# bxh1/VIDO-SLAM

Hardware: AMD Instinct MI355X
Metric: frames/sec end-to-end (flow+depth+track+local-BA) at 640x480; BA iters/sec (higher is better)
Workload: dtype f32

## Files before the change

vido-slam_amd/csrc/conv3x3h.hip:

```cpp
#include "common.hpp"
#include <type_traits>

namespace {
typedef float f32x16 __attribute__((ext_vector_type(16)));
typedef float f32x2 __attribute__((ext_vector_type(2)));
typedef _Float16 f16x8 __attribute__((ext_vector_type(8)));
typedef _Float16 f16x2 __attribute__((ext_vector_type(2)));
typedef unsigned u32x4 __attribute__((ext_vector_type(4)));

#define C3_OOB 0x40000000u
#define C3_WSLOT 24576
#define C3_RBW 3
#define C3_WPIX(BR) (((BR) + 2) * 18)
#define C3_XP(BR) ((16 * C3_WPIX(BR) + 511) / 512)
#define C3_RAW(BR) (C3_XP(BR) * 8 * 256)
#define C3_PLANE(BR) (C3_WPIX(BR) * 32)
#define C3_PBUF(BR) (2 * C3_PLANE(BR))
#define C3_LDS(BR) (C3_RBW * C3_WSLOT + C3_RAW(BR) + 2 * C3_PBUF(BR))

struct C3Args { const float* x; const void* wp; const float* bias; float* y; int N, Cin, Cout, H, W, nby, nbx, mt, total, nchunk; float slope; unsigned wbytes; unsigned* range_flag; };

template <int RPW, int CG>
__global__ __launch_bounds__(512) void k_conv3x3_h(C3Args A)
{
    constexpr int BR = 16 / CG, MT = 32 * RPW * CG, WPIX = C3_WPIX(BR), XP = C3_XP(BR), RAWB = C3_RAW(BR), PLANE = C3_PLANE(BR), PBUF = C3_PBUF(BR), CK = (WPIX * 8 + 511) / 512, NMM = 9 * RPW, NRD = 2 * RPW + 2;
    extern __shared__ __attribute__((aligned(16))) char c3_lds[];
    char* L = c3_lds;
    const int tid = threadIdx.x, lane = tid & 63, w = __builtin_amdgcn_readfirstlane(tid >> 6);
    const int per = gridDim.x >> 3, item = (blockIdx.x & 7) * per + (blockIdx.x >> 3);
    if (item >= A.total) return;
    const int nt = item / A.mt, mtile = item - nt * A.mt, m0 = mtile * MT;
    const int bpi = A.nby * A.nbx, n = nt / bpi, brem = nt - n * bpi, by = brem / A.nbx, bx = brem - by * A.nbx, Y0 = by * BR, X0 = bx * 16;
    const int rp = CG == 1 ? w : (w & 3), rb0 = CG == 1 ? 0 : RPW * (w >> 2);
    const int hw = A.H * A.W, nsteps = A.nchunk * 3;

    const __amdgpu_buffer_rsrc_t wr = __builtin_amdgcn_make_buffer_rsrc((void*)A.wp, 0, A.wbytes, 0x00020000);
    const unsigned avo = 16u * (unsigned)lane;
    unsigned abase[3], avq[3];
#pragma unroll
    for (int q = 0; q < 3; q++) { const int i = w + 8 * q, rb = i / 6, rem = i - 6 * rb; abase[q] = 1024u * (unsigned)(((m0 >> 5) + rb) * A.nchunk * 18 + rem); avq[q] = rb < RPW * CG ? avo : 0x80000000u; }
    unsigned xvo[11];
#pragma unroll
    for (int j = 0; j < XP; j++) {
        const int e = 64 * (8 * j + w) + lane, ch = e / WPIX, rem = e - ch * WPIX, row = rem / 18, col = rem - row * 18, gy = Y0 - 1 + row, gx = X0 - 1 + col;
        xvo[j] = (e < 16 * WPIX && gy >= 0 && gy < A.H && gx >= 0 && gx < A.W) ? 4u * (unsigned)(ch * hw + gy * A.W + gx) : C3_OOB;
    }
    const unsigned ximg = 4u * (unsigned)n * (unsigned)A.Cin * (unsigned)hw, ximg_end = ximg + 4u * (unsigned)A.Cin * (unsigned)hw, xchunk = 64u * (unsigned)hw;
    char* const RAW = L + C3_RBW * C3_WSLOT;
    char* const PL = RAW + RAWB;
    auto issue_w = [&](int s, int slot) {
        char* S = L + slot * C3_WSLOT + w * 1024;
        const unsigned so = 6144u * (unsigned)s;
#pragma unroll
        for (int q = 0; q < 3; q++) __builtin_amdgcn_raw_ptr_buffer_load_lds(wr, (__attribute__((address_space(3))) void*)(S + q * 8192), 16, avq[q], abase[q] + so, 0, 0);
    };
    auto issue_x = [&](int c) {
        const unsigned so = ximg + xchunk * (unsigned)c;
        const __amdgpu_buffer_rsrc_t xc = __builtin_amdgcn_make_buffer_rsrc((void*)((const char*)A.x + so), 0, ximg_end - so, 0x00020000);
#pragma unroll
        for (int j = 0; j < XP; j++) __builtin_amdgcn_raw_ptr_buffer_load_lds(xc, (__attribute__((address_space(3))) void*)(RAW + (8 * j + w) * 256), 4, xvo[j], 0, 0, 0);
    };
    float xmax = 0.f;
    const f32x2 k2048 = {2048.f, 2048.f};
    auto convert = [&](int buf) {
        const float* R = (const float*)RAW;
        unsigned* P = (unsigned*)(PL + buf * PBUF);
#pragma unroll
        for (int k = 0; k < CK; k++) {
            const int idx = tid + 512 * k;
            if (k < CK - 1 || idx < WPIX * 8) {
                const int q = idx / WPIX, pix = idx - q * WPIX;
                const f32x2 v = {R[(2 * q) * WPIX + pix], R[(2 * q + 1) * WPIX + pix]};
                const f16x2 h = __builtin_convertvector(v, f16x2);
                f32x2 vs, r;
                asm("v_pk_mul_f32 %0, %1, %2" : "=v"(vs) : "v"(v), "v"(k2048));
                asm("v_fma_mix_f32 %0, %1, %2, %3 op_sel_hi:[1,0,0]" : "=v"(r.x) : "v"(h), "s"(-2048.f), "v"(vs.x));
                asm("v_fma_mix_f32 %0, %1, %2, %3 op_sel:[1,0,0] op_sel_hi:[1,0,0]" : "=v"(r.y) : "v"(h), "s"(-2048.f), "v"(vs.y));
                const f16x2 l = __builtin_convertvector(r, f16x2);
                P[pix * 8 + q] = __builtin_bit_cast(unsigned, h); P[PLANE / 4 + pix * 8 + q] = __builtin_bit_cast(unsigned, l);
                xmax = __builtin_elementwise_maximum(__builtin_elementwise_maximum(xmax, __builtin_fabsf(v.x)), __builtin_fabsf(v.y));
            }
        }
    };

    f32x16 acc[RPW], acl[RPW];
#pragma unroll
    for (int rb = 0; rb < RPW; rb++)
#pragma unroll
        for (int r = 0; r < 16; r++) { acc[rb][r] = 0.f; acl[rb][r] = 0.f; }
    typedef const __attribute__((address_space(3))) char* lds_c;
    const unsigned a_lane = 16u * (unsigned)lane;
    const unsigned b_lane = (unsigned)(C3_RBW * C3_WSLOT + RAWB) + 32u * (unsigned)((2 * rp + ((lane & 31) >> 4)) * 18 + (lane & 15)) + 16u * (unsigned)(lane >> 5);

    issue_x(0); issue_w(0, 0); issue_w(min(1, nsteps - 1), 1);
    asm volatile("s_waitcnt vmcnt(6) lgkmcnt(0)\n\ts_barrier" ::: "memory");
    convert(0);
    int slot = 0;
    u32x4 a[2][RPW][2], b[2][2];
    auto step = [&](auto dy_c, auto nbuf_c, int pbuf, auto&& copies) {
        constexpr int dy = decltype(dy_c)::value, NBUF = decltype(nbuf_c)::value;
        lds_c Ab = (lds_c)(L + slot * C3_WSLOT) + a_lane;
        lds_c Bb = (lds_c)L + b_lane + pbuf * PBUF + dy * (18 * 32);
        auto ld = [&](int dx, int set) {
#pragma unroll
            for (int rb = 0; rb < RPW; rb++)
#pragma unroll
                for (int pl = 0; pl < 2; pl++) a[set][rb][pl] = *(const __attribute__((address_space(3))) u32x4*)(Ab + (((rb0 + rb) * 3 + dx) * 2 + pl) * 1024);
#pragma unroll
            for (int pl = 0; pl < 2; pl++) b[set][pl] = *(const __attribute__((address_space(3))) u32x4*)(Bb + dx * 32 + pl * PLANE);
        };
        __builtin_amdgcn_sched_barrier(0);
        ld(0, 0);
        copies();
#pragma unroll
        for (int dx = 0; dx < 3; dx++) {
            if (dx < 2) ld(dx + 1, (dx + 1) & 1);
#pragma unroll
            for (int term = 0; term < 3; term++) {
                constexpr int PA[3] = {0, 1, 0}, PB[3] = {1, 0, 0};
#pragma unroll
                for (int rb = 0; rb < RPW; rb++) {
                    f32x16& d = term == 2 ? acc[rb] : acl[rb];
                    d = __builtin_amdgcn_mfma_f32_32x32x16_f16(__builtin_bit_cast(f16x8, a[dx & 1][rb][PA[term]]), __builtin_bit_cast(f16x8, b[dx & 1][PB[term]]), d, 0, 0, 0);
                }
            }
        }
        __builtin_amdgcn_sched_group_barrier(0x100, NRD, 0);
#pragma unroll
        for (int i = 0; i < NMM; i++) {
            __builtin_amdgcn_sched_group_barrier(0x008, 1, 0);
            if (i < 2 * NRD) __builtin_amdgcn_sched_group_barrier(0x100, 1, 0);
            if (i >= 1 && i < 1 + NBUF) __builtin_amdgcn_sched_group_barrier(0x020, 1, 0);
        }
        __builtin_amdgcn_sched_barrier(0);
    };
    for (int c = 0; c < A.nchunk; c++) {
        const int pbuf = c & 1, cn = min(c + 1, A.nchunk - 1);
        asm volatile("s_waitcnt vmcnt(3) lgkmcnt(0)\n\ts_barrier" ::: "memory");
        step(std::integral_constant<int, 0>{}, std::integral_constant<int, 3 + XP>{}, pbuf, [&] { const int sf = slot == 0 ? C3_RBW - 1 : slot - 1; issue_w(min(3 * c + 2, nsteps - 1), sf); issue_x(cn); });
        slot = slot + 1 == C3_RBW ? 0 : slot + 1;
        asm volatile("s_waitcnt vmcnt(%0) lgkmcnt(0)\n\ts_barrier" :: "n"(3 + XP) : "memory");
        step(std::integral_constant<int, 1>{}, std::integral_constant<int, 3>{}, pbuf, [&] { const int sf = slot == 0 ? C3_RBW - 1 : slot - 1; issue_w(min(3 * c + 3, nsteps - 1), sf); });
        slot = slot + 1 == C3_RBW ? 0 : slot + 1;
        asm volatile("s_waitcnt vmcnt(3) lgkmcnt(0)\n\ts_barrier" ::: "memory");
        step(std::integral_constant<int, 2>{}, std::integral_constant<int, 3>{}, pbuf, [&] { const int sf = slot == 0 ? C3_RBW - 1 : slot - 1; issue_w(min(3 * c + 4, nsteps - 1), sf); });
        convert(pbuf ^ 1);
        slot = slot + 1 == C3_RBW ? 0 : slot + 1;
    }
    asm volatile("s_waitcnt vmcnt(0) lgkmcnt(0)" ::: "memory");
#pragma unroll
    for (int rb = 0; rb < RPW; rb++) acc[rb] += acl[rb] * 0x1p-11f;
    if (!(xmax < 65504.f) && A.range_flag) atomicOr(A.range_flag, 1u);

    const float* wsc = (const float*)((const char*)A.wp + (size_t)A.nchunk * 16 * 18 * A.Cout * 2);
    const int p = lane & 31, Y = Y0 + 2 * rp + (p >> 4), X = X0 + (p & 15);
    const bool inside = Y < A.H && X < A.W;
    float* yb = A.y + (size_t)n * A.Cout * hw + (size_t)Y * A.W + X;
#pragma unroll
    for (int rb = 0; rb < RPW; rb++) {
        float bv[16], sv[16];
#pragma unroll
        for (int r = 0; r < 16; r++) { const int co = m0 + 32 * (rb0 + rb) + 8 * (r >> 2) + 4 * (lane >> 5) + (r & 3); bv[r] = A.bias ? A.bias[co] : 0.f; sv[r] = wsc[co]; }
        if (inside) {
#pragma unroll
            for (int r = 0; r < 16; r++) {
                const int co = m0 + 32 * (rb0 + rb) + 8 * (r >> 2) + 4 * (lane >> 5) + (r & 3);
                const float v = acc[rb][r] * sv[r] + bv[r];
                yb[(size_t)co * hw] = fmaxf(v, v * A.slope);
            }
        }
    }
}
}

extern "C" {

int vido_conv3x3_h_supported(int n, int cin, int cout, int h, int w)
{
    const long long cp = (cin + 15) / 16 * 16;
    return n >= 1 && cin >= 1 && (cout == 32 || cout == 64 || (cout >= 128 && cout % 128 == 0)) && h >= 1 && w >= 1 && 4ll * n * cin * h * w < (1ll << 30) && 4ll * n * cout * h * w < (1ll << 30)
           && 36ll * cp * cout < (1ll << 31);
}

#define C3_MIN16 190
static int c3_block_rows(int n, int cout, int h, int w)
{
    static const int force = [] { const char* e = getenv("VIDO_CONV3X3_H_ROWS"); return e ? atoi(e) : 0; }();
    if (cout == 32) return 16;
    if (force == 16 || force == 8) return force;
    const int mt = cout >= 128 ? cout / 128 : 1;
    return n * ((h + 15) / 16) * ((w + 15) / 16) * mt >= C3_MIN16 ? 16 : 8;
}
int vido_conv3x3_h_workgroups(int n, int cout, int h, int w) { const int br = c3_block_rows(n, cout, h, w); return n * ((h + br - 1) / br) * ((w + 15) / 16) * (cout >= 128 ? cout / 128 : 1); }

int vido_conv3x3_h_bias_act(vido_ctx* ctx, const float* x, const void* w_packed, const float* bias, float* y, int n, int cin, int cout, int h, int w, float slope)
{
    if (!ctx) return VIDO_E_INVALID;
    if (!x || !w_packed || !y || x == y || !vido_conv3x3_h_supported(n, cin, cout, h, w) || slope < 0.f || slope > 1.f || (((uintptr_t)x | (uintptr_t)y) & 3) || ((uintptr_t)w_packed & 15))
        return vido_set_error(ctx, VIDO_E_INVALID, "conv3x3_h: no kernel for %d x %d -> %d channels at %d x %d (or a pointer is misaligned, or slope outside [0, 1])", n, cin, cout, h, w);
    HIP_TRY(ctx, hipSetDevice(ctx->device));
    hipStream_t st = ctx->has_ext_stream ? ctx->ext_stream : ctx->stream;
    const int br = c3_block_rows(n, cout, h, w);
    const int nby = (h + br - 1) / br, nbx = (w + 15) / 16, mt = cout >= 128 ? cout / 128 : 1, total = n * nby * nbx * mt;
    const int nchunk = (cin + 15) / 16;
    C3Args A{x, w_packed, bias, y, n, cin, cout, h, w, nby, nbx, mt, total, nchunk, slope, (unsigned)(36ll * 16 * nchunk * cout), ctx->c1_range_flag};
    static bool attr[64] = {};
    if (!attr[ctx->device & 63]) {
#define C3_ATTR(RPW_, CG_) HIP_TRY(ctx, hipFuncSetAttribute((const void*)k_conv3x3_h<RPW_, CG_>, hipFuncAttributeMaxDynamicSharedMemorySize, (int)C3_LDS(16 / CG_)))
        C3_ATTR(4, 1); C3_ATTR(2, 2); C3_ATTR(2, 1); C3_ATTR(1, 2); C3_ATTR(1, 1);
#undef C3_ATTR
        attr[ctx->device & 63] = true;
    }
    const dim3 grid(8 * ((total + 7) / 8));
#define C3_LAUNCH(RPW_, CG_) hipLaunchKernelGGL((k_conv3x3_h<RPW_, CG_>), grid, dim3(512), C3_LDS(16 / CG_), st, A)
    if (cout >= 128) { if (br == 16) C3_LAUNCH(4, 1); else C3_LAUNCH(2, 2); }
    else if (cout == 64) { if (br == 16) C3_LAUNCH(2, 1); else C3_LAUNCH(1, 2); }
    else C3_LAUNCH(1, 1);
#undef C3_LAUNCH
    HIP_TRY(ctx, hipGetLastError());
    return VIDO_OK;
}

}
```

Before: 125.0.

## Load conv input via registers and stage whole 3x3 weight chunks per slot

Input chunks no longer go through a raw f32 LDS staging area. They are loaded with buffer loads straight into registers and converted to the split f16 hi/lo planes, with 128-bit LDS stores. For the smaller output-tile variants the weight ring now holds all three dy rows of a chunk per slot, so a chunk needs one barrier instead of three. Ring depth is derived per template from an LDS budget. The aim is to cut LDS traffic, barriers and LDS footprint, at the cost of more registers held live across the MFMA loop and different waitcnt accounting.

Measured after the change: 127.2, median of 6. 1.7% higher.

```diff
diff --git a/vido-slam_amd/csrc/conv3x3h.hip b/vido-slam_amd/csrc/conv3x3h.hip
--- a/vido-slam_amd/csrc/conv3x3h.hip
+++ b/vido-slam_amd/csrc/conv3x3h.hip
@@ -9,21 +9,27 @@
 typedef unsigned u32x4 __attribute__((ext_vector_type(4)));
 
 #define C3_OOB 0x40000000u
-#define C3_WSLOT 24576
-#define C3_RBW 3
-#define C3_WPIX(BR) (((BR) + 2) * 18)
-#define C3_XP(BR) ((16 * C3_WPIX(BR) + 511) / 512)
-#define C3_RAW(BR) (C3_XP(BR) * 8 * 256)
-#define C3_PLANE(BR) (C3_WPIX(BR) * 32)
-#define C3_PBUF(BR) (2 * C3_PLANE(BR))
-#define C3_LDS(BR) (C3_RBW * C3_WSLOT + C3_RAW(BR) + 2 * C3_PBUF(BR))
+#ifndef C3_RING128
+#define C3_RING128 3
+#endif
+template <int RPW, int CG> struct C3Form {
+    static constexpr int BR = 16 / CG, RB = RPW * CG, DS = RB == 4 ? 1 : 3;
+    static constexpr int PPR = 6 * DS, QW = (RB * PPR + 7) / 8, WSLOT = 8 * QW * 1024;
+    static constexpr int WPIX = (BR + 2) * 18, PLANE = WPIX * 32, PBUF = 2 * PLANE;
+    static constexpr int XI = (2 * WPIX + 511) / 512, XL = 8 * XI;
+    static constexpr int RBW = DS == 1 ? C3_RING128 : (3 * WSLOT + 2 * PBUF <= 160 * 1024 ? 3 : 2);
+    static constexpr int LDS = RBW * WSLOT + 2 * PBUF;
+    static_assert(LDS <= 160 * 1024 && QW <= 5 && XI <= 2, "conv3x3_h: LDS, register arrays");
+};
 
 struct C3Args { const float* x; const void* wp; const float* bias; float* y; int N, Cin, Cout, H, W, nby, nbx, mt, total, nchunk; float slope; unsigned wbytes; unsigned* range_flag; };
 
 template <int RPW, int CG>
 __global__ __launch_bounds__(512) void k_conv3x3_h(C3Args A)
 {
-    constexpr int BR = 16 / CG, MT = 32 * RPW * CG, WPIX = C3_WPIX(BR), XP = C3_XP(BR), RAWB = C3_RAW(BR), PLANE = C3_PLANE(BR), PBUF = C3_PBUF(BR), CK = (WPIX * 8 + 511) / 512, NMM = 9 * RPW, NRD = 2 * RPW + 2;
+    typedef C3Form<RPW, CG> F;
+    constexpr int BR = F::BR, MT = 32 * RPW * CG, DS = F::DS, PPR = F::PPR, QW = F::QW, WSLOT = F::WSLOT, RBW = F::RBW, PD = RBW - 1;
+    constexpr int WPIX = F::WPIX, PLANE = F::PLANE, PBUF = F::PBUF, XI = F::XI, XL = F::XL, NMM = 9 * RPW, NRD = 2 * RPW + 2;
     extern __shared__ __attribute__((aligned(16))) char c3_lds[];
     char* L = c3_lds;
     const int tid = threadIdx.x, lane = tid & 63, w = __builtin_amdgcn_readfirstlane(tid >> 6);
@@ -32,53 +38,59 @@
     const int nt = item / A.mt, mtile = item - nt * A.mt, m0 = mtile * MT;
     const int bpi = A.nby * A.nbx, n = nt / bpi, brem = nt - n * bpi, by = brem / A.nbx, bx = brem - by * A.nbx, Y0 = by * BR, X0 = bx * 16;
     const int rp = CG == 1 ? w : (w & 3), rb0 = CG == 1 ? 0 : RPW * (w >> 2);
-    const int hw = A.H * A.W, nsteps = A.nchunk * 3;
+    const int hw = A.H * A.W, nsteps = A.nchunk * (3 / DS);
 
     const __amdgpu_buffer_rsrc_t wr = __builtin_amdgcn_make_buffer_rsrc((void*)A.wp, 0, A.wbytes, 0x00020000);
     const unsigned avo = 16u * (unsigned)lane;
-    unsigned abase[3], avq[3];
-#pragma unroll
-    for (int q = 0; q < 3; q++) { const int i = w + 8 * q, rb = i / 6, rem = i - 6 * rb; abase[q] = 1024u * (unsigned)(((m0 >> 5) + rb) * A.nchunk * 18 + rem); avq[q] = rb < RPW * CG ? avo : 0x80000000u; }
-    unsigned xvo[11];
-#pragma unroll
-    for (int j = 0; j < XP; j++) {
-        const int e = 64 * (8 * j + w) + lane, ch = e / WPIX, rem = e - ch * WPIX, row = rem / 18, col = rem - row * 18, gy = Y0 - 1 + row, gx = X0 - 1 + col;
-        xvo[j] = (e < 16 * WPIX && gy >= 0 && gy < A.H && gx >= 0 && gx < A.W) ? 4u * (unsigned)(ch * hw + gy * A.W + gx) : C3_OOB;
+    unsigned abase[5], avq[5];
+#pragma unroll
+    for (int q = 0; q < QW; q++) { const int i = w + 8 * q, rb = i / PPR, rem = i - PPR * rb; abase[q] = 1024u * (unsigned)(((m0 >> 5) + rb) * A.nchunk * 18 + rem); avq[q] = rb < RPW * CG ? avo : 0x80000000u; }
+    unsigned xo[2], xs[2];
+#pragma unroll
+    for (int k = 0; k < XI; k++) {
+        const int e = tid + 512 * k, hh = e / WPIX, pix = e - hh * WPIX, row = pix / 18, col = pix - row * 18, gy = Y0 - 1 + row, gx = X0 - 1 + col;
+        const bool in = hh < 2 && gy >= 0 && gy < A.H && gx >= 0 && gx < A.W;
+        xo[k] = in ? 4u * (unsigned)(8 * hh * hw + gy * A.W + gx) : C3_OOB; xs[k] = in ? 4u * (unsigned)hw : 0u;
     }
     const unsigned ximg = 4u * (unsigned)n * (unsigned)A.Cin * (unsigned)hw, ximg_end = ximg + 4u * (unsigned)A.Cin * (unsigned)hw, xchunk = 64u * (unsigned)hw;
-    char* const RAW = L + C3_RBW * C3_WSLOT;
-    char* const PL = RAW + RAWB;
+    char* const PL = L + RBW * WSLOT;
     auto issue_w = [&](int s, int slot) {
-        char* S = L + slot * C3_WSLOT + w * 1024;
-        const unsigned so = 6144u * (unsigned)s;
-#pragma unroll
-        for (int q = 0; q < 3; q++) __builtin_amdgcn_raw_ptr_buffer_load_lds(wr, (__attribute__((address_space(3))) void*)(S + q * 8192), 16, avq[q], abase[q] + so, 0, 0);
-    };
+        char* S = L + slot * WSLOT + w * 1024;
+        const unsigned so = 1024u * PPR * (unsigned)s;
+#pragma unroll
+        for (int q = 0; q < QW; q++) __builtin_amdgcn_raw_ptr_buffer_load_lds(wr, (__attribute__((address_space(3))) void*)(S + q * 8192), 16, avq[q], abase[q] + so, 0, 0);
+    };
+    float xv[2][8];
     auto issue_x = [&](int c) {
         const unsigned so = ximg + xchunk * (unsigned)c;
         const __amdgpu_buffer_rsrc_t xc = __builtin_amdgcn_make_buffer_rsrc((void*)((const char*)A.x + so), 0, ximg_end - so, 0x00020000);
 #pragma unroll
-        for (int j = 0; j < XP; j++) __builtin_amdgcn_raw_ptr_buffer_load_lds(xc, (__attribute__((address_space(3))) void*)(RAW + (8 * j + w) * 256), 4, xvo[j], 0, 0, 0);
+        for (int k = 0; k < XI; k++)
+#pragma unroll
+            for (int j = 0; j < 8; j++) xv[k][j] = __builtin_bit_cast(float, __builtin_amdgcn_raw_buffer_load_b32(xc, xo[k] + (unsigned)j * xs[k], 0, 0));
     };
     float xmax = 0.f;
     const f32x2 k2048 = {2048.f, 2048.f};
     auto convert = [&](int buf) {
-        const float* R = (const float*)RAW;
-        unsigned* P = (unsigned*)(PL + buf * PBUF);
-#pragma unroll
-        for (int k = 0; k < CK; k++) {
-            const int idx = tid + 512 * k;
-            if (k < CK - 1 || idx < WPIX * 8) {
-                const int q = idx / WPIX, pix = idx - q * WPIX;
-                const f32x2 v = {R[(2 * q) * WPIX + pix], R[(2 * q + 1) * WPIX + pix]};
-                const f16x2 h = __builtin_convertvector(v, f16x2);
-                f32x2 vs, r;
-                asm("v_pk_mul_f32 %0, %1, %2" : "=v"(vs) : "v"(v), "v"(k2048));
-                asm("v_fma_mix_f32 %0, %1, %2, %3 op_sel_hi:[1,0,0]" : "=v"(r.x) : "v"(h), "s"(-2048.f), "v"(vs.x));
-                asm("v_fma_mix_f32 %0, %1, %2, %3 op_sel:[1,0,0] op_sel_hi:[1,0,0]" : "=v"(r.y) : "v"(h), "s"(-2048.f), "v"(vs.y));
-                const f16x2 l = __builtin_convertvector(r, f16x2);
-                P[pix * 8 + q] = __builtin_bit_cast(unsigned, h); P[PLANE / 4 + pix * 8 + q] = __builtin_bit_cast(unsigned, l);
-                xmax = __builtin_elementwise_maximum(__builtin_elementwise_maximum(xmax, __builtin_fabsf(v.x)), __builtin_fabsf(v.y));
+        char* P = PL + buf * PBUF;
+#pragma unroll
+        for (int k = 0; k < XI; k++) {
+            const int e = tid + 512 * k, hh = e / WPIX, pix = e - hh * WPIX;
+            {
+                u32x4 hv, lv;
+#pragma unroll
+                for (int j = 0; j < 4; j++) {
+                    const f32x2 v = {xv[k][2 * j], xv[k][2 * j + 1]};
+                    const f16x2 h = __builtin_convertvector(v, f16x2);
+                    f32x2 vs, r;
+                    asm("v_pk_mul_f32 %0, %1, %2" : "=v"(vs) : "v"(v), "v"(k2048));
+                    asm("v_fma_mix_f32 %0, %1, %2, %3 op_sel_hi:[1,0,0]" : "=v"(r.x) : "v"(h), "s"(-2048.f), "v"(vs.x));
+                    asm("v_fma_mix_f32 %0, %1, %2, %3 op_sel:[1,0,0] op_sel_hi:[1,0,0]" : "=v"(r.y) : "v"(h), "s"(-2048.f), "v"(vs.y));
+                    const f16x2 l = __builtin_convertvector(r, f16x2);
+                    hv[j] = __builtin_bit_cast(unsigned, h); lv[j] = __builtin_bit_cast(unsigned, l);
+                    xmax = __builtin_elementwise_maximum(__builtin_elementwise_maximum(xmax, __builtin_fabsf(v.x)), __builtin_fabsf(v.y));
+                }
+                if (k < XI - 1 || e < 2 * WPIX) { *(u32x4*)(P + pix * 32 + hh * 16) = hv; *(u32x4*)(P + PLANE + pix * 32 + hh * 16) = lv; }
             }
         }
     };
@@ -90,22 +102,23 @@
         for (int r = 0; r < 16; r++) { acc[rb][r] = 0.f; acl[rb][r] = 0.f; }
     typedef const __attribute__((address_space(3))) char* lds_c;
     const unsigned a_lane = 16u * (unsigned)lane;
-    const unsigned b_lane = (unsigned)(C3_RBW * C3_WSLOT + RAWB) + 32u * (unsigned)((2 * rp + ((lane & 31) >> 4)) * 18 + (lane & 15)) + 16u * (unsigned)(lane >> 5);
-
-    issue_x(0); issue_w(0, 0); issue_w(min(1, nsteps - 1), 1);
-    asm volatile("s_waitcnt vmcnt(6) lgkmcnt(0)\n\ts_barrier" ::: "memory");
+    const unsigned b_lane = (unsigned)(RBW * WSLOT) + 32u * (unsigned)((2 * rp + ((lane & 31) >> 4)) * 18 + (lane & 15)) + 16u * (unsigned)(lane >> 5);
+
+    issue_x(0);
+#pragma unroll
+    for (int s = 0; s < PD; s++) issue_w(min(s, nsteps - 1), s);
     convert(0);
     int slot = 0;
     u32x4 a[2][RPW][2], b[2][2];
-    auto step = [&](auto dy_c, auto nbuf_c, int pbuf, auto&& copies) {
+    auto taps = [&](auto dy_c, auto nbuf_c, int pbuf, auto&& copies) {
         constexpr int dy = decltype(dy_c)::value, NBUF = decltype(nbuf_c)::value;
-        lds_c Ab = (lds_c)(L + slot * C3_WSLOT) + a_lane;
+        lds_c Ab = (lds_c)(L + slot * WSLOT) + a_lane + (DS == 3 ? dy * 6 * 1024 : 0);
         lds_c Bb = (lds_c)L + b_lane + pbuf * PBUF + dy * (18 * 32);
         auto ld = [&](int dx, int set) {
 #pragma unroll
             for (int rb = 0; rb < RPW; rb++)
 #pragma unroll
-                for (int pl = 0; pl < 2; pl++) a[set][rb][pl] = *(const __attribute__((address_space(3))) u32x4*)(Ab + (((rb0 + rb) * 3 + dx) * 2 + pl) * 1024);
+                for (int pl = 0; pl < 2; pl++) a[set][rb][pl] = *(const __attribute__((address_space(3))) u32x4*)(Ab + ((rb0 + rb) * PPR + dx * 2 + pl) * 1024);
 #pragma unroll
             for (int pl = 0; pl < 2; pl++) b[set][pl] = *(const __attribute__((address_space(3))) u32x4*)(Bb + dx * 32 + pl * PLANE);
         };
@@ -134,18 +147,31 @@
         }
         __builtin_amdgcn_sched_barrier(0);
     };
+    auto next_slot = [&] { slot = slot + 1 == RBW ? 0 : slot + 1; };
+    auto issue_ahead = [&](int s) { issue_w(min(s + PD, nsteps - 1), slot == 0 ? RBW - 1 : slot - 1); };
+    typedef std::integral_constant<int, 0> I0;
+    typedef std::integral_constant<int, 1> I1;
+    typedef std::integral_constant<int, 2> I2;
     for (int c = 0; c < A.nchunk; c++) {
         const int pbuf = c & 1, cn = min(c + 1, A.nchunk - 1);
-        asm volatile("s_waitcnt vmcnt(3) lgkmcnt(0)\n\ts_barrier" ::: "memory");
-        step(std::integral_constant<int, 0>{}, std::integral_constant<int, 3 + XP>{}, pbuf, [&] { const int sf = slot == 0 ? C3_RBW - 1 : slot - 1; issue_w(min(3 * c + 2, nsteps - 1), sf); issue_x(cn); });
-        slot = slot + 1 == C3_RBW ? 0 : slot + 1;
-        asm volatile("s_waitcnt vmcnt(%0) lgkmcnt(0)\n\ts_barrier" :: "n"(3 + XP) : "memory");
-        step(std::integral_constant<int, 1>{}, std::integral_constant<int, 3>{}, pbuf, [&] { const int sf = slot == 0 ? C3_RBW - 1 : slot - 1; issue_w(min(3 * c + 3, nsteps - 1), sf); });
-        slot = slot + 1 == C3_RBW ? 0 : slot + 1;
-        asm volatile("s_waitcnt vmcnt(3) lgkmcnt(0)\n\ts_barrier" ::: "memory");
-        step(std::integral_constant<int, 2>{}, std::integral_constant<int, 3>{}, pbuf, [&] { const int sf = slot == 0 ? C3_RBW - 1 : slot - 1; issue_w(min(3 * c + 4, nsteps - 1), sf); });
+        if constexpr (DS == 1) {
+            asm volatile("s_waitcnt vmcnt(%0) lgkmcnt(0)\n\ts_barrier" :: "n"((PD - 1) * QW) : "memory");
+            taps(I0{}, std::integral_constant<int, XL + QW>{}, pbuf, [&] { issue_x(cn); issue_ahead(3 * c); });
+            next_slot();
+            asm volatile("s_waitcnt vmcnt(%0) lgkmcnt(0)\n\ts_barrier" :: "n"((PD - 1) * QW + (PD > 1 ? XL : 0)) : "memory");
+            taps(I1{}, std::integral_constant<int, QW>{}, pbuf, [&] { issue_ahead(3 * c + 1); });
+            next_slot();
+            asm volatile("s_waitcnt vmcnt(%0) lgkmcnt(0)\n\ts_barrier" :: "n"((PD - 1) * QW + (PD > 2 ? XL : 0)) : "memory");
+            taps(I2{}, std::integral_constant<int, QW>{}, pbuf, [&] { issue_ahead(3 * c + 2); });
+            next_slot();
+        } else {
+            asm volatile("s_waitcnt vmcnt(%0) lgkmcnt(0)\n\ts_barrier" :: "n"((PD - 1) * QW) : "memory");
+            taps(I0{}, std::integral_constant<int, XL + (PD == 1 ? QW : 0)>{}, pbuf, [&] { issue_x(cn); if (PD == 1) issue_ahead(c); });
+            taps(I1{}, std::integral_constant<int, PD == 1 ? 0 : QW>{}, pbuf, [&] { if (PD > 1) issue_ahead(c); });
+            taps(I2{}, std::integral_constant<int, 0>{}, pbuf, [] {});
+            next_slot();
+        }
         convert(pbuf ^ 1);
-        slot = slot + 1 == C3_RBW ? 0 : slot + 1;
     }
     asm volatile("s_waitcnt vmcnt(0) lgkmcnt(0)" ::: "memory");
 #pragma unroll
@@ -206,13 +232,13 @@
     C3Args A{x, w_packed, bias, y, n, cin, cout, h, w, nby, nbx, mt, total, nchunk, slope, (unsigned)(36ll * 16 * nchunk * cout), ctx->c1_range_flag};
     static bool attr[64] = {};
     if (!attr[ctx->device & 63]) {
-#define C3_ATTR(RPW_, CG_) HIP_TRY(ctx, hipFuncSetAttribute((const void*)k_conv3x3_h<RPW_, CG_>, hipFuncAttributeMaxDynamicSharedMemorySize, (int)C3_LDS(16 / CG_)))
+#define C3_ATTR(RPW_, CG_) HIP_TRY(ctx, hipFuncSetAttribute((const void*)k_conv3x3_h<RPW_, CG_>, hipFuncAttributeMaxDynamicSharedMemorySize, (C3Form<RPW_, CG_>::LDS)))
         C3_ATTR(4, 1); C3_ATTR(2, 2); C3_ATTR(2, 1); C3_ATTR(1, 2); C3_ATTR(1, 1);
 #undef C3_ATTR
         attr[ctx->device & 63] = true;
     }
     const dim3 grid(8 * ((total + 7) / 8));
-#define C3_LAUNCH(RPW_, CG_) hipLaunchKernelGGL((k_conv3x3_h<RPW_, CG_>), grid, dim3(512), C3_LDS(16 / CG_), st, A)
+#define C3_LAUNCH(RPW_, CG_) hipLaunchKernelGGL((k_conv3x3_h<RPW_, CG_>), grid, dim3(512), (C3Form<RPW_, CG_>::LDS), st, A)
     if (cout >= 128) { if (br == 16) C3_LAUNCH(4, 1); else C3_LAUNCH(2, 2); }
     else if (cout == 64) { if (br == 16) C3_LAUNCH(2, 1); else C3_LAUNCH(1, 2); }
     else C3_LAUNCH(1, 1);
```
